# legend-exp/dspeed

Hardware: AMD Instinct MI355X
Metric: waveforms/sec, 4096-sample fp32 trap-energy chain (higher is better)
Workload: dtype f32; 1 GPU; 1000000 x 4096 float32 rows per GPU, fused bl_subtract->pole_zero(tau=1716.28)->trap_filter(625,188)->fixed_time_pickoff('l'); BASELINE configs[1]; rows_per_gpu=1000000, wf_len=4096, device= (gfx950:sramecc+:xnack-), entry=build_processing_chain, kernel=dsp_energy_rr_kernel, lds_bytes_per_wave=19696, waves_per_block=4, blocks=512

## Files before the change

### dspeed_amd/build.py

```python
from __future__ import annotations

import os
import shutil
import subprocess
import sys

HERE = os.path.dirname(os.path.abspath(__file__))
CSRC = os.path.join(HERE, "csrc")
LIB = os.path.join(HERE, "libdspeed_hip.so")
LIB_DIAG = os.path.join(HERE, "libdspeed_hip_diag.so")
SOURCES = ["dsp_vm.hip", "dsp_energy.hip", "dsp_fit.hip", "dsp_rows.hip", "dsp_current.hip", "dsp_scalar.hip", "dsp_reduce.hip", "dsp_pz.hip", "dsp_fir_mfma.hip", "dsp_fir_f16.hip", "dsp_fir_runs.hip", "dsp_plan.cpp", "dsp_host.cpp"]
DEPS = SOURCES + ["dsp_program.h", "dsp_plan.h", "dsp_wave.h", "dsp_reduce_tail.h", os.path.join("..", "..", "include", "dspeed_hip.h")]
FLAGS = ["--offload-arch=gfx950", "-O3", "-std=c++17", "-ffp-contract=off", "-fno-fast-math", "-fPIC", "-shared", "-Wall",
         "-Wno-unused-function"]


NO_SCRATCH = {"dsp_vm.hip": "dsp_vm_kernel"}


def _check_scratch(src: str, remarks: str) -> None:
    frag, name, bad = NO_SCRATCH[src], None, []
    for line in remarks.splitlines():
        if "Function Name:" in line:
            name = line.split("Function Name:")[1].split()[0]
        elif "ScratchSize [bytes/lane]:" in line and name and frag in name:
            n = int(line.split("ScratchSize [bytes/lane]:")[1].split()[0])
            if n:
                bad.append((name, n))
    skip = 0
    for line in remarks.splitlines():
        if "remark:" in line:
            skip = 2
        elif skip and (line.lstrip()[:1].isdigit() or line.lstrip().startswith("|")):
            skip -= 1
        else:
            skip = 0
            sys.stderr.write(line + "\n")
    if bad:
        raise RuntimeError(f"{src}: scratch memory in " + ", ".join(f"{n} ({b} B/lane)" for n, b in bad) +
                           " -- a helper taking Ctx& was outlined, or a local array is indexed at run time (see NO_SCRATCH in build.py)")


def _hipcc() -> str:
    for cand in (os.environ.get("HIPCC"), shutil.which("hipcc"), "/opt/rocm/bin/hipcc"):
        if cand and os.path.exists(cand):
            return cand
    raise RuntimeError("hipcc not found (need ROCm)")


def _stamp(diag: bool) -> str:
    import hashlib

    h = hashlib.sha256(repr((FLAGS, sorted(NO_SCRATCH.items()), diag)).encode())
    for d in DEPS:
        with open(os.path.join(CSRC, d), "rb") as f:
            h.update(d.encode() + b"\0" + f.read())
    return h.hexdigest()


def _stamp_file(lib: str) -> str:
    return lib + ".stamp"


def needs_build(lib: str = LIB) -> bool:
    if not os.path.exists(lib) or not os.path.exists(_stamp_file(lib)):
        return True
    with open(_stamp_file(lib)) as f:
        return f.read().strip() != _stamp(lib == LIB_DIAG)


def build(force: bool = False, verbose: bool = False, diag: bool = False, variant: str | None = None, defines=(), extra_flags=()) -> str:
    lib = LIB_DIAG if diag else LIB
    if variant:
        lib = os.path.join(HERE, f"libdspeed_hip_{variant}.so")
        force = True
    if not force and not needs_build(lib):
        return lib
    objs, procs = [], []
    for src in SOURCES:
        obj = os.path.join(CSRC, "." + src + (f".{variant}.o" if variant else (".diag.o" if diag else ".o")))
        cmd = [_hipcc(), *[f for f in FLAGS if f != "-shared"], *(["-DDSPEED_HIP_DIAG"] if diag else []), *[f"-D{d}" for d in defines], *extra_flags, "-x", "hip", "-c",
               os.path.join(CSRC, src), "-o", obj]
        guard = src in NO_SCRATCH
        if guard:
            cmd.append("-Rpass-analysis=kernel-resource-usage")
        if verbose:
            print(" ".join(cmd))
        procs.append((cmd, subprocess.Popen(cmd, stderr=subprocess.PIPE if guard else None, text=True if guard else None), src))
        objs.append(obj)
    failed = None
    try:
        for cmd, p, src in procs:
            err = p.communicate()[1] if src in NO_SCRATCH else None
            if p.wait() != 0:
                if err:
                    sys.stderr.write(err)
                raise subprocess.CalledProcessError(p.returncode, cmd)
            if err is not None:
                _check_scratch(src, err)
    except BaseException as e:
        failed = e
    if failed is not None:
        for _cmd, p, _src in procs:
            if p.poll() is None:
                p.kill()
            p.wait()
        for obj in objs:
            if os.path.exists(obj):
                os.remove(obj)
        raise failed
    link = [_hipcc(), "--offload-arch=gfx950", "-fPIC", "-shared", *objs, "-o", lib]
    if verbose:
        print(" ".join(link))
    subprocess.check_call(link)
    if variant:
        for obj in objs:
            os.remove(obj)
        return lib
    with open(_stamp_file(lib), "w") as f:
        f.write(_stamp(diag) + "\n")
    return lib


if __name__ == "__main__":
    _variant = sys.argv[sys.argv.index("--variant") + 1] if "--variant" in sys.argv else None
    _defines = [sys.argv[i + 1] for i, a in enumerate(sys.argv[:-1]) if a == "--define"]
    _flags = [sys.argv[i + 1] for i, a in enumerate(sys.argv[:-1]) if a == "--flag"]
    print(build(force="--force" in sys.argv, verbose=True, diag="--diag" in sys.argv, variant=_variant, defines=_defines, extra_flags=_flags))
```

### dspeed_amd/csrc/dsp_energy.hip

```cpp
#include <hip/hip_runtime.h>

#include "dsp_program.h"
#include "dsp_wave.h"

struct EnergyArgs {
    const void* wf;
    int64_t wf_stride;
    int32_t wf_offset;
    int32_t len;
    const float* bl;
    int64_t bl_stride;
    float bl_const;
    int32_t has_bl;
    const float* tp;
    int64_t tp_stride;
    float tp_const;
    int32_t mode;
    float* out;
    int64_t out_stride;
    double c;
    double rr, ll;
    int32_t tau_nan;
    int32_t all_nan;
    int32_t C, pitch;
    float invC;
    int32_t q[3], rho[3];
    int32_t lds_elems_per_wave;
    int32_t slot_off;
    const float* tau;
    int64_t tau_stride;
    int32_t ablate;
};

#ifdef DSPEED_HIP_DIAG
#define ABLATE(A) ((A).ablate)
#else
#define ABLATE(A) 0
#endif

constexpr int rr_prio_after_phase[6] = {1, 2, 3, 3, 3, 0};
#define RR_PRIO_AT(n) __builtin_amdgcn_s_setprio(rr_prio_after_phase[n]);

namespace {

constexpr int G = 8;
constexpr int G3 = 8;

__device__ __forceinline__ unsigned long long stamp() {
    unsigned long long t;
    __builtin_amdgcn_sched_barrier(0);
    asm volatile("s_memtime %0\n\ts_waitcnt lgkmcnt(0)" : "=s"(t)::"memory");
    __builtin_amdgcn_sched_barrier(0);
    return t;
}
#define PHASE(i)                                   \
    if (stamps) {                                  \
        const unsigned long long now_ = stamp();   \
        tsum[i] += now_ - tlast;                   \
        tlast = now_;                              \
    }

template <int N>
__device__ __forceinline__ void load_group(float (&v)[N], const float* p) {
#pragma unroll
    for (int u = 0; u < N; ++u) v[u] = p[u];
}

template <int NPF, int KIND>
__global__ void __launch_bounds__(256, 2) dsp_energy_kernel(EnergyArgs A, int64_t n_wf, int* err) {
    extern __shared__ __attribute__((aligned(16))) unsigned char smem_raw[];
    const int lane = lane_id();
    const double inv_rr = 1.0 / A.rr, inv_ll = 1.0 / A.ll;
    const int wave = __builtin_amdgcn_readfirstlane((int)(threadIdx.x >> 6)), wpb = (int)(blockDim.x >> 6);
    float* lds = reinterpret_cast<float*>(smem_raw) + (size_t)wave * A.lds_elems_per_wave;
    for (int e = lane; e < A.lds_elems_per_wave; e += 64) lds[e] = 0.0f;
    wave_sync();

    constexpr int C = 4 * NPF, pitch = C + 1, len = 256 * NPF;
    float* slot = lds + A.slot_off;
    float* mine = slot + lane * pitch;

    const float* lagp[3];
#pragma unroll
    for (int k = 0; k < 3; ++k) {
        const int jj = lane - A.q[k] - 1;
        lagp[k] = (jj >= -1) ? slot + jj * pitch + (C - A.rho[k]) : slot - 2 * pitch;
    }

    const int64_t stride_rows = (int64_t)gridDim.x * wpb;
    int64_t row = (int64_t)blockIdx.x * wpb + wave;

    typedef float f4 __attribute__((ext_vector_type(4)));
    f4 pf[NPF];
    float pf_bl = 0.0f, pf_tp = 0.0f;
    auto prefetch = [&](int64_t r) {
        const float* g = (const float*)A.wf + r * A.wf_stride + A.wf_offset;
#pragma unroll
        for (int b = 0; b < NPF; ++b) pf[b] = reinterpret_cast<const f4*>(g)[b * 64 + lane];
        pf_bl = A.bl ? A.bl[r * A.bl_stride] : A.bl_const;
        pf_tp = A.tp ? A.tp[r * A.tp_stride] : A.tp_const;
    };
    auto report = [&](int code, int64_t r) {
        if (lane == 0 && atomicCAS(&err[0], 0, code) == 0) {
            err[1] = (int)(r & 0xffffffffll);
            err[2] = (int)(r >> 32);
        }
    };
    if (row < n_wf) prefetch(row);
    const bool stamps = (ABLATE(A) & 8) != 0;
    unsigned long long tsum[6] = {0, 0, 0, 0, 0, 0}, tlast = stamps ? stamp() : 0;

    for (; row < n_wf; row += stride_rows) {
#pragma unroll
        for (int b = 0; b < NPF; ++b) {
            const int e = (b * 64 + lane) * 4;
            float* d = slot + e + e / C;
#pragma unroll
            for (int m = 0; m < 4; ++m) d[m] = pf[b][m];
        }
        const float bl = __int_as_float(__builtin_amdgcn_readfirstlane(__float_as_int(pf_bl)));
        const float t_in = __int_as_float(__builtin_amdgcn_readfirstlane(__float_as_int(pf_tp)));
        const int64_t next = row + stride_rows;
        __builtin_amdgcn_sched_barrier(0);
        if (next < n_wf) prefetch(next);
        __builtin_amdgcn_sched_barrier(0);
        wave_sync();
        PHASE(0)

        float result = quiet_nan<float>();
        double X = 0.0;
        if (!(ABLATE(A) & 1)) {
            float va[G], vb[G];
            load_group(va, mine);
#pragma unroll 1
            for (int t = 0; t < C; t += 2 * G) {
                load_group(vb, mine + t + G);
#pragma unroll
                for (int u = 0; u < G; ++u) X += (double)(va[u] - bl);
                if (t + 2 * G < C) load_group(va, mine + t + 2 * G);
#pragma unroll
                for (int u = 0; u < G; ++u) X += (double)(vb[u] - bl);
            }
        }
// ... 95 lines not shown
                for (int k = 0; k < 4; ++k)
                    if (co[k] >= 0) capmask |= 1u << (co[k] / G3);
                PHASE(3)
                float y = g;
                {
                    float a0[G3], a1[G3], a2[G3], a3[G3], b0[G3], b1[G3], b2[G3], b3[G3];
                    auto fetch = [&](float (&o)[G3], float (&l0)[G3], float (&l1)[G3], float (&l2)[G3], int t) {
                        load_group(o, mine + t);
#pragma unroll
                        for (int k = 0; k < 3; ++k) {
                            float(&dst)[G3] = (k == 0) ? l0 : (k == 1 ? l1 : l2);
                            const int r = A.rho[k];
                            if (t >= r) {
                                load_group(dst, lagp[k] + t + 1);
                            } else if (t + G3 <= r) {
                                load_group(dst, lagp[k] + t);
                            } else {
#pragma unroll
                                for (int u = 0; u < G3; ++u) dst[u] = lagp[k][t + u + ((t + u >= r) ? 1 : 0)];
                            }
                        }
                    };
                    auto body = [&](float (&o)[G3], float (&l0)[G3], float (&l1)[G3], float (&l2)[G3], int t) {
                        float ys[G3];
#pragma unroll
                        for (int u = 0; u < G3; ++u) {
                            y = trap_step_r<float, KIND>(y, o[u], l0[u], l1[u], l2[u], A.rr, A.ll, inv_rr, inv_ll);
                            ys[u] = y;
                        }
                        if ((capmask >> (t / G3)) & 1u) {
#pragma unroll
                            for (int k = 0; k < 4; ++k) {
                                const int d = co[k] - t;
#pragma unroll
                                for (int u = 0; u < G3; ++u)
                                    if (d == u) capv[k] = ys[u];
                            }
                        }
                    };
                    fetch(a0, a1, a2, a3, 0);
#pragma unroll 1
                    for (int t = 0; t < C; t += 2 * G3) {
                        fetch(b0, b1, b2, b3, t + G3);
                        body(a0, a1, a2, a3, t);
                        if (t + 2 * G3 < C) fetch(a0, a1, a2, a3, t + 2 * G3);
                        body(b0, b1, b2, b3, t + G3);
                    }
                }
                PHASE(4)
                const double D = (double)y - (double)g;
                const double delta = wave_exscan_add(D) - (double)g;
                float w4[4];
#pragma unroll
                for (int k = 0; k < 4; ++k) {
                    const float v = (float)((double)capv[k] + delta);
                    w4[k] = cl[k] >= 0 ? readlane(v, cl[k]) : 0.0f;
                }
                int fc = 0;
                result = pickoff_eval(t_in, A.mode, len, w4, fc);
                if (fc) report(fc, row);
            }
        }
        if (lane == 0) A.out[row * A.out_stride] = result;
        wave_sync();
        PHASE(5)
    }
    if (stamps && lane == 0) {
#pragma unroll
        for (int i = 0; i < 6; ++i) atomicAdd(reinterpret_cast<unsigned long long*>(err + 4) + i, tsum[i]);
    }
}

struct EnergyPlan {
    int32_t shift[3][4];
    int32_t cs[3][4];
    int32_t local[3][4];
};

__device__ __attribute__((noinline)) double rr_decay(double tau) { return exp(-1.0 / tau); }

template <int NPF, int KIND, int S, int IN, bool TAU = false>
__global__ void __launch_bounds__(256, NPF >= 32 ? 1 : 2) dsp_energy_rr_kernel(EnergyArgs A, EnergyPlan PL, int64_t n_wf, int* err) {
    extern __shared__ __attribute__((aligned(16))) unsigned char smem_raw[];
    constexpr int C = 4 * NPF + 1, len = 256 * NPF, NG = (C - 1) / 8, CS = (C - 1) / S, NGS = CS / 8;
    constexpr int BS = CS >= 16 ? 16 : CS;
    static_assert((C - 1) % (8 * S) == 0, "sub-chain length must be a whole number of 8-sample groups");
    const int lane = lane_id();
    const double inv_rr = 1.0 / A.rr, inv_ll = 1.0 / A.ll;
    const int wave = __builtin_amdgcn_readfirstlane((int)(threadIdx.x >> 6)), wpb = (int)(blockDim.x >> 6);
    float* lds = reinterpret_cast<float*>(smem_raw) + (size_t)wave * A.lds_elems_per_wave;
    for (int e = lane; e < A.lds_elems_per_wave; e += 64) lds[e] = 0.0f;
    wave_sync();
    float* slot = lds + A.slot_off;
    float* mine = slot + lane * C;
    constexpr int AUXP = NG + 1 <= 9 ? 9 : ((NG + 1) | 1);
    static_assert(NG + 1 <= AUXP && S * NGS + 1 <= AUXP && (AUXP & 1) == 1, "side array too small");
    float* aux = slot + 64 * C + 16 + lane * AUXP;
    const float* lagp[3];
#pragma unroll
    for (int k = 0; k < 3; ++k) {
        const int pos0 = lane * C - A.q[k];
        lagp[k] = (pos0 >= -C) ? slot + pos0 : slot - (2 * C + 8);
    }

    const int64_t stride_rows = (int64_t)gridDim.x * wpb;
    int64_t row = (int64_t)blockIdx.x * wpb + wave;
    typedef float f4 __attribute__((ext_vector_type(4)));
    typedef unsigned int u4 __attribute__((ext_vector_type(4)));
    constexpr int NLD = IN == 0 ? NPF : NPF / 2;
    static_assert(IN == 0 || NPF % 2 == 0, "16-bit rows: an even number of 4-sample groups per lane");
    u4 pf[NLD];
    float pf_bl = 0.0f, pf_tp = 0.0f;
    auto prefetch = [&](int64_t r) {
        const char* g = (const char*)A.wf + (r * A.wf_stride + A.wf_offset) * (IN == 0 ? 4 : 2);
#pragma unroll
        for (int b = 0; b < NLD; ++b) pf[b] = reinterpret_cast<const u4*>(g)[b * 64 + lane];
        typedef const __attribute__((address_space(1))) float* gptr;
        pf_bl = A.bl ? ((gptr)A.bl)[r * A.bl_stride] : A.bl_const;
        pf_tp = A.tp ? ((gptr)A.tp)[r * A.tp_stride] : A.tp_const;
    };
    auto report = [&](int code, int64_t r) {
        if (lane == 0 && atomicCAS(&err[0], 0, code) == 0) {
            err[1] = (int)(r & 0xffffffffll);
            err[2] = (int)(r >> 32);
        }
    };
    if (row < n_wf) prefetch(row);
    const bool stamps = (ABLATE(A) & 8) != 0;
    unsigned long long tsum[6] = {0, 0, 0, 0, 0, 0}, tlast = stamps ? stamp() : 0;
    float pend_result = 0.0f;
    int64_t pend_row = -1;

    for (; row < n_wf; row += stride_rows) {
#pragma unroll
        for (int b = 0; b < NLD; ++b) {
            if (IN == 0) {
                f4 v;
#pragma unroll
                for (int m = 0; m < 4; ++m) v[m] = __uint_as_float(pf[b][m]);
                *reinterpret_cast<f4*>(slot + (b * 64 + lane) * 4) = v - pf_bl;
            } else {
                f4 lo, hi;
#pragma unroll
                for (int m = 0; m < 4; ++m) {
                    const unsigned int wv = pf[b][m];
                    const float s0 = IN == 1 ? (float)(short)(wv & 0xffffu) : (float)(wv & 0xffffu);
                    const float s1 = IN == 1 ? (float)(short)(wv >> 16) : (float)(wv >> 16);
                    if (m < 2) {
                        lo[2 * m] = s0;
                        lo[2 * m + 1] = s1;
                    } else {
                        hi[2 * (m - 2)] = s0;
                        hi[2 * (m - 2) + 1] = s1;
                    }
                }
                *reinterpret_cast<f4*>(slot + (b * 64 + lane) * 8) = lo - pf_bl;
                *reinterpret_cast<f4*>(slot + (b * 64 + lane) * 8 + 4) = hi - pf_bl;
            }
        }
        slot[len + lane] = 0.0f;
        const float t_in = __int_as_float(__builtin_amdgcn_readfirstlane(__float_as_int(pf_tp)));
        const int64_t next = row + stride_rows;
        __builtin_amdgcn_sched_barrier(0);
        if (next < n_wf) prefetch(next);
        if (pend_row >= 0 && lane == 0) A.out[pend_row * A.out_stride] = pend_result;
        __builtin_amdgcn_sched_barrier(0);
        wave_sync();
        PHASE(0)
        RR_PRIO_AT(0)

        float result = quiet_nan<float>();
        float xr[C];
#pragma unroll
        for (int t = 0; t < C; ++t) xr[t] = mine[t];
        const float xprev = (lane > 0) ? mine[-1] : 0.0f;
        double Xp[4] = {0.0, 0.0, 0.0, 0.0};
#pragma unroll
        for (int t = 0; t < C; ++t) {
            if ((t & 7) == 0) __builtin_amdgcn_sched_barrier(0);
            Xp[t & 3] += (double)xr[t];
        }
        const double X = (Xp[0] + Xp[1]) + (Xp[2] + Xp[3]);
        double c_row = A.c;
        bool in_nan = A.tau_nan != 0;
        if constexpr (TAU) {
            const float tau = A.tau[row * A.tau_stride];
            in_nan = tau != tau;
            c_row = rr_decay((double)tau);
        }
        if (wave_any(!(fabs(X) <= 1.7976931348623157e308))) {
            bool n = false;
#pragma unroll
            for (int t = 0; t < C; ++t) n |= (xr[t] != xr[t]);
            in_nan |= wave_any(n);
        }
        PHASE(1)
        RR_PRIO_AT(1)
#pragma unroll
        for (int t = 0; t < C; ++t) asm volatile("" : "+v"(xr[t]));
        if (!in_nan) {
            const double E = wave_exscan_add(X);
            const double c = c_row;
            double xp = (double)xprev, acc = E - c * (E - xp);
            float run = 0.0f;
#pragma unroll
            for (int t = 0; t < C; ++t) {
                if ((t & 7) == 0) __builtin_amdgcn_sched_barrier(0);
                const double x = (double)xr[t];
                acc += __builtin_fma(-c, xp, x);
                const float y = (float)acc;
                xr[t] = y;
                mine[t] = y;
                xp = x;
                run += y;
                if ((t & 7) == 7) aux[t >> 3] = run;
            }
            wave_sync();
            PHASE(2)
        RR_PRIO_AT(2)
            bool pz_nan = false;
            if (wave_any(!(fabsf(run) <= 3.4028234663852886e38f))) {
                bool n = false;
#pragma unroll
                for (int t = 0; t < C; ++t) n |= (xr[t] != xr[t]);
                pz_nan = wave_any(n);
            }
            if (pz_nan) {
                report(DSP_E_PZ_NAN, row);
            } else if (!A.all_nan && !(ABLATE(A) & 4) && pickoff_in_range(t_in, len)) {
                const double Ep = wave_exscan_add((double)run);
                float g[S], y[S];
#pragma unroll
                for (int s = 0; s < S; ++s) {
                    double Ak[3];
                    float pbase[3], pv[3][8];
                    int pn[3];
#pragma unroll
                    for (int k = 0; k < 3; ++k) {
                        int r = PL.cs[k][s] * CS + PL.local[k][s];
                        asm volatile("" : "+s"(r));
                        const int gi = (r > 0 ? r - 1 : 0) >> 3;
                        pn[k] = r - 8 * gi;
                        const float b = aux[gi > 0 ? gi - 1 : 0];
                        pbase[k] = gi > 0 ? b : 0.0f;
                        const float* p = mine + 8 * gi;
#pragma unroll
                        for (int u = 0; u < 8; ++u) pv[k][u] = p[u];
                    }
#pragma unroll
                    for (int k = 0; k < 3; ++k) {
                        float part = 0.0f;
#pragma unroll
                        for (int u = 0; u < 8; ++u) part += (u < pn[k]) ? pv[k][u] : 0.0f;
                        Ak[k] = wave_shift_up(Ep + (double)(pbase[k] + part), PL.shift[k][s]);
                    }
                    const double own = Ep + (s ? (double)aux[s * NGS - 1] : 0.0);
                    double Gd;
                    if (KIND == TRAP_FILTER)
                        Gd = ((own - Ak[0]) - Ak[1]) + Ak[2];
                    else if (KIND == TRAP_NORM)
                        Gd = (((own - Ak[0]) - Ak[1]) + Ak[2]) / A.rr;
                    else
                        Gd = (own - Ak[0]) / A.rr - (Ak[1] - Ak[2]) / A.ll;
                    g[s] = (lane == 0 && s == 0) ? -0.0f : (float)Gd;
                    y[s] = g[s];
                }
                PHASE(3)
        RR_PRIO_AT(3)
                wave_sync();
                const int i0 = (int)t_in;
                int capst[2], capoff[2], caplane[2];
#pragma unroll
                for (int k = 0; k < 2; ++k) {
                    const int e = i0 + k;
                    const bool ok = e >= 0 && e < len;
                    caplane[k] = ok ? e / C : 0;
                    capoff[k] = ok ? e - caplane[k] * C : 0;
                    capst[k] = ok ? capoff[k] / BS : -1;
                }
                int capmask = (capst[0] >= 0 ? 1 << capst[0] : 0) | (capst[1] >= 0 ? 1 << capst[1] : 0);
                asm volatile("" : "+s"(capmask));
                float* capbuf = slot + 64 * C + 16 + 64 * AUXP;
                float ysb[S][BS];
                constexpr int GL = 4, NL = CS / GL;
                constexpr int PD = S == 1 ? 2 : 1;
                float lb[PD + 1][S][GL][3], lodd[3] = {0.0f, 0.0f, 0.0f};
#pragma unroll
                for (int p = 0; p < PD; ++p)
#pragma unroll
                    for (int s = 0; s < S; ++s)
#pragma unroll
                        for (int u = 0; u < GL; ++u)
#pragma unroll
                            for (int k = 0; k < 3; ++k) lb[p][s][u][k] = lagp[k][s * CS + p * GL + u];
#pragma unroll
                for (int gl = 0; gl < NL; ++gl) {
                    __builtin_amdgcn_sched_barrier(0);
                    if (gl + PD < NL) {
#pragma unroll
                        for (int s = 0; s < S; ++s)
#pragma unroll
                            for (int u = 0; u < GL; ++u)
#pragma unroll
                                for (int k = 0; k < 3; ++k) lb[(gl + PD) % (PD + 1)][s][u][k] = lagp[k][s * CS + (gl + PD) * GL + u];
                    } else if (gl + PD == NL) {
#pragma unroll
                        for (int k = 0; k < 3; ++k) lodd[k] = lagp[k][C - 1];
                    }
                    if ((gl * GL) % 8 == 0) {
#pragma unroll
                        for (int s = 0; s < S; ++s) aux[s * NGS + (gl * GL) / 8] = y[s];
                    }
                    __builtin_amdgcn_sched_barrier(0);
#pragma unroll
                    for (int u = 0; u < GL; ++u)
#pragma unroll
                        for (int s = 0; s < S; ++s) {
                            y[s] = trap_step_r<float, KIND>(y[s], xr[s * CS + gl * GL + u], lb[gl % (PD + 1)][s][u][0], lb[gl % (PD + 1)][s][u][1],
                                                          lb[gl % (PD + 1)][s][u][2], A.rr, A.ll, inv_rr, inv_ll);
                            ysb[s][(gl * GL + u) % BS] = y[s];
                        }
                    if (((gl + 1) * GL) % BS == 0) {
#pragma unroll
                        for (int s = 0; s < S; ++s) {
                            const int q = s * (CS / BS) + (gl * GL) / BS;
                            if (capmask & (1 << q)) {
#pragma unroll
                                for (int k = 0; k < 2; ++k)
                                    if (capst[k] == q && lane == caplane[k]) {
#pragma unroll
                                        for (int u = 0; u < BS; ++u) capbuf[k * 16 + u] = ysb[s][u];
                                    }
                            }
                        }
                    }
                }
                aux[S * NGS] = y[S - 1];
                y[S - 1] = trap_step_r<float, KIND>(y[S - 1], xr[C - 1], lodd[0], lodd[1], lodd[2], A.rr, A.ll, inv_rr, inv_ll);
                PHASE(4)
        RR_PRIO_AT(4)
                double D[S], Dbefore[S], Dtot = 0.0;
#pragma unroll
                for (int s = 0; s < S; ++s) {
                    D[s] = (double)y[s] - (double)g[s];
                    Dbefore[s] = Dtot;
                    Dtot += D[s];
                }
                const double T0 = wave_exscan_add(Dtot);
                const bool wide = (A.mode == 'h');
                float w4[4];
#pragma unroll
                for (int k = 0; k < 2; ++k) {
                    float v = capbuf[k * 16 + (capoff[k] % BS)];
                    v = capoff[k] == C - 1 ? y[S - 1] : v;
                    double delta = T0 - (double)g[0];
#pragma unroll
                    for (int s = 1; s < S; ++s)
                        if (capoff[k] >= s * CS) delta = (T0 + Dbefore[s]) - (double)g[s];
                    w4[1 + k] = capst[k] >= 0 ? readlane((float)((double)v + delta), caplane[k]) : 0.0f;
                }
#pragma unroll
                for (int k = 0; k < 4; k += 3) {
                    const int e = i0 - 1 + k;
                    const bool need = wide && e >= 0 && e < len;
                    w4[k] = 0.0f;
                    __builtin_amdgcn_sched_barrier(0);
                    if (need) {
                        const int l = e / C, off = e - l * C;
                        int ch = off / CS;
                        if (ch > S - 1) ch = S - 1;
                        const int loc = off - ch * CS;
                        const int gi = loc >> 3, u0 = loc & 7;
                        float ys = aux[ch * NGS + gi], gsel = 0.0f;
                        double dsel = 0.0;
#pragma unroll
                        for (int s = 0; s < S; ++s)
                            if (ch == s) {
                                gsel = g[s];
                                dsel = Dbefore[s];
                            }
                        const int base = ch * CS + gi * 8;
                        float yk = ys;
#pragma unroll
                        for (int u = 0; u < 8; ++u) {
                            const int tt = base + u;
                            ys = trap_step_r<float, KIND>(ys, mine[tt], lagp[0][tt], lagp[1][tt], lagp[2][tt], A.rr, A.ll, inv_rr, inv_ll);
                            if (u == u0) yk = ys;
                        }
                        const double delta = (T0 + dsel) - (double)gsel;
                        w4[k] = readlane((float)((double)yk + delta), l);
                    }
                }
                int fc = 0;
                result = pickoff_eval(t_in, A.mode, len, w4, fc);
                if (fc) report(fc, row);
            }
        }
        pend_result = result;
        pend_row = row;
        wave_sync();
        PHASE(5)
        RR_PRIO_AT(5)
    }
    if (pend_row >= 0 && lane == 0) A.out[pend_row * A.out_stride] = pend_result;
    if (stamps && lane == 0) {
#pragma unroll
        for (int i = 0; i < 6; ++i) atomicAdd(reinterpret_cast<unsigned long long*>(err + 4) + i, tsum[i]);
    }
}

template <int KIND, int S, int IN, bool TAU = false>
int launch_rr_kind(const EnergyArgs& A, const EnergyPlan& PL, int npf, int64_t n_wf, int* err, int blocks, int threads, int lds_bytes,
                   hipStream_t st) {
    switch (npf) {
        case 4: hipLaunchKernelGGL((dsp_energy_rr_kernel<4, KIND, S, IN, TAU>), dim3(blocks), dim3(threads), lds_bytes, st, A, PL, n_wf, err); break;
        case 8: hipLaunchKernelGGL((dsp_energy_rr_kernel<8, KIND, S, IN, TAU>), dim3(blocks), dim3(threads), lds_bytes, st, A, PL, n_wf, err); break;
        case 16: hipLaunchKernelGGL((dsp_energy_rr_kernel<16, KIND, S, IN, TAU>), dim3(blocks), dim3(threads), lds_bytes, st, A, PL, n_wf, err); break;
        case 32:
            if (S != 1) return (int)hipErrorInvalidValue;
            hipLaunchKernelGGL((dsp_energy_rr_kernel<32, KIND, 1, IN, TAU>), dim3(blocks), dim3(threads), lds_bytes, st, A, PL, n_wf, err);
            break;
        default: return (int)hipErrorInvalidValue;
    }
    return (int)hipGetLastError();
}

template <int KIND>
int launch_kind(const EnergyArgs& A, int npf, int64_t n_wf, int* err, int blocks, int threads, int lds_bytes, hipStream_t s) {
    switch (npf) {
        case 4: hipLaunchKernelGGL((dsp_energy_kernel<4, KIND>), dim3(blocks), dim3(threads), lds_bytes, s, A, n_wf, err); break;
        case 8: hipLaunchKernelGGL((dsp_energy_kernel<8, KIND>), dim3(blocks), dim3(threads), lds_bytes, s, A, n_wf, err); break;
        case 16: hipLaunchKernelGGL((dsp_energy_kernel<16, KIND>), dim3(blocks), dim3(threads), lds_bytes, s, A, n_wf, err); break;
        case 32: hipLaunchKernelGGL((dsp_energy_kernel<32, KIND>), dim3(blocks), dim3(threads), lds_bytes, s, A, n_wf, err); break;
        default: return (int)hipErrorInvalidValue;
    }
    return (int)hipGetLastError();
}

}

extern "C" int dsp_internal_launch_energy(const EnergyArgs* A, int trap_opcode, int npf, int64_t n_wf, int* err, int blocks,
                                          int threads, int lds_bytes, hipStream_t stream) {
    if (trap_opcode == DSP_OP_TRAP_FILTER) return launch_kind<TRAP_FILTER>(*A, npf, n_wf, err, blocks, threads, lds_bytes, stream);
    if (trap_opcode == DSP_OP_TRAP_NORM) return launch_kind<TRAP_NORM>(*A, npf, n_wf, err, blocks, threads, lds_bytes, stream);
    return launch_kind<TRAP_ASYM>(*A, npf, n_wf, err, blocks, threads, lds_bytes, stream);
}

extern "C" int dsp_internal_set_energy_lds(int trap_opcode, int npf, int lds_bytes) {
#define SET_(NPF, KIND)                                                                                                   \
    if (npf == NPF && kind == KIND)                                                                                        \
        return (int)hipFuncSetAttribute(reinterpret_cast<const void*>(&dsp_energy_kernel<NPF, KIND>),                      \
                                        hipFuncAttributeMaxDynamicSharedMemorySize, lds_bytes);
    const int kind = trap_opcode == DSP_OP_TRAP_FILTER ? TRAP_FILTER : (trap_opcode == DSP_OP_TRAP_NORM ? TRAP_NORM : TRAP_ASYM);
    SET_(4, TRAP_FILTER) SET_(8, TRAP_FILTER) SET_(16, TRAP_FILTER) SET_(32, TRAP_FILTER)
    SET_(4, TRAP_NORM) SET_(8, TRAP_NORM) SET_(16, TRAP_NORM) SET_(32, TRAP_NORM)
    SET_(4, TRAP_ASYM) SET_(8, TRAP_ASYM) SET_(16, TRAP_ASYM) SET_(32, TRAP_ASYM)
#undef SET_
    return (int)hipErrorInvalidValue;
}

extern "C" int dsp_internal_launch_energy_rr(const EnergyArgs* A, const EnergyPlan* PL, int trap_opcode, int npf, int S, int wf_dtype,
                                             int64_t n_wf, int* err, int blocks, int threads, int lds_bytes, hipStream_t stream) {
#define GO_(KIND)                                                                                                          \
    if (A->tau && wf_dtype == DSP_I16) return launch_rr_kind<KIND, 1, 1, true>(*A, *PL, npf, n_wf, err, blocks, threads, lds_bytes, stream); \
    if (A->tau && wf_dtype == DSP_U16) return launch_rr_kind<KIND, 1, 2, true>(*A, *PL, npf, n_wf, err, blocks, threads, lds_bytes, stream); \
    if (A->tau) return launch_rr_kind<KIND, 1, 0, true>(*A, *PL, npf, n_wf, err, blocks, threads, lds_bytes, stream);       \
    if (wf_dtype == DSP_I16) return launch_rr_kind<KIND, 1, 1>(*A, *PL, npf, n_wf, err, blocks, threads, lds_bytes, stream); \
    if (wf_dtype == DSP_U16) return launch_rr_kind<KIND, 1, 2>(*A, *PL, npf, n_wf, err, blocks, threads, lds_bytes, stream); \
    return S == 2 ? launch_rr_kind<KIND, 2, 0>(*A, *PL, npf, n_wf, err, blocks, threads, lds_bytes, stream)                \
// ... 10 lines not shown
```

### dspeed_amd/csrc/dsp_plan.cpp

```cpp
#include "dsp_plan.h"

#include <algorithm>
#include <cmath>
#include <cstdarg>
#include <cstdio>
#include <cstdlib>
#include <cstring>
#include <memory>
#include <vector>

namespace {
thread_local std::string g_last_error;
}

int dsp_fail(int code, const char* fmt, ...) {
    char buf[512];
    va_list ap;
    va_start(ap, fmt);
    vsnprintf(buf, sizeof buf, fmt, ap);
    va_end(ap);
    g_last_error = buf;
    return code;
}
void dsp_set_last_error(const char* text) { g_last_error = text ? text : ""; }
// ... 1257 lines not shown
        }
    }
    P.n_ops = n_dev_ops;

    {
        int i = 0;
        const dsp_op* ld = (n_ops > i && ops[i].opcode == DSP_OP_LOAD) ? &ops[i++] : nullptr;
        const dsp_op* bs = (ld && n_ops > i && ops[i].opcode == DSP_OP_BL_SUBTRACT) ? &ops[i++] : nullptr;
        const dsp_op* pz = (ld && n_ops > i && ops[i].opcode == DSP_OP_POLE_ZERO) ? &ops[i++] : nullptr;
        const dsp_op* tp = (pz && n_ops > i && ops[i].opcode == DSP_OP_TRAP_PICKOFF) ? &ops[i++] : nullptr;
        const dsp_op* st = (tp && n_ops > i && ops[i].opcode == DSP_OP_STORE_SCALAR) ? &ops[i++] : nullptr;
        const int wdt = ld ? io[ld->io].dtype : -1;
        const bool tau_col = pz && pz->sp[0].kind == DSP_ARG_INPUT && io[pz->sp[0].index].dtype == DSP_F32;
        const bool shape = !f64 && st && i == n_ops && n_slots == 1 && ld->ip[0] == 0 && ld->ip[1] == 0 && (wdt == DSP_F32 || wdt == DSP_I16 || wdt == DSP_U16) && P.io[ld->io].vec_ok &&
                           (!bs || (bs->dst == 0 && bs->src == 0 && bs->sp[0].kind != DSP_ARG_REG)) && pz->dst == 0 && pz->src == 0 &&
                           (pz->sp[0].kind == DSP_ARG_CONST || tau_col) &&
                           tp->src == 0 && tp->sp[0].kind != DSP_ARG_REG && st->ip[0] == tp->dst &&
                           (slot_len[0] == 1024 || slot_len[0] == 2048 || slot_len[0] == 4096 || slot_len[0] == 8192);
        if (!shape && st && i == n_ops && n_slots == 1) {
            if (f64) note(ch, "the energy chain in a float64 loop: the fused energy kernels are float32");
            else if (pz->sp[0].kind != DSP_ARG_CONST && !tau_col)
                note(ch, "a pole-zero time constant per event that is not a float32 column: the fused energy kernels take a constant or such a column");
            else if (!(slot_len[0] == 1024 || slot_len[0] == 2048 || slot_len[0] == 4096 || slot_len[0] == 8192))
                note(ch, "waveforms of %d samples: the fused energy kernels take 1024, 2048, 4096 or 8192", slot_len[0]);
            else if (!P.io[ld->io].vec_ok) note(ch, "rows that do not start on 16-byte boundaries: the fused energy kernels read 16 bytes per lane");
        }
        auto f32_col = [&](const dsp_scalar_arg& a) { return a.kind != DSP_ARG_INPUT || io[a.index].dtype == DSP_F32; };
        if (shape && (!bs || f32_col(bs->sp[0])) && f32_col(tp->sp[0]) && io[st->io].dtype == DSP_F32) {
            EnergyArgs& F = ch->fused;
            const DevOp& dpz = P.ops[dev_index[pz - ops]];
            const DevOp& dtp = P.ops[dev_index[tp - ops]];
            F.wf_stride = io[ld->io].row_stride;
            F.wf_offset = io[ld->io].offset;
            F.len = slot_len[0];
            F.has_bl = bs ? 1 : 0;
            if (bs) {
                if (bs->sp[0].kind == DSP_ARG_INPUT) {
                    ch->io_bl = bs->sp[0].index;
                    F.bl_stride = io[ch->io_bl].row_stride;
                } else {
                    F.bl_const = (float)bs->sp[0].value;
                }
            }
            if (tp->sp[0].kind == DSP_ARG_INPUT) {
                ch->io_tp = tp->sp[0].index;
                F.tp_stride = io[ch->io_tp].row_stride;
            } else {
                F.tp_const = (float)tp->sp[0].value;
            }
            F.mode = tp->io;
            F.out_stride = io[st->io].row_stride;
            F.c = dpz.fc[0];
            F.tau_nan = dpz.ic[0];
            F.rr = dtp.fc[0];
            F.ll = dtp.fc[1];
            F.all_nan = dtp.ic[9];
            F.C = P.slots[0].C;
            F.pitch = P.slots[0].pitch;
            F.invC = P.slots[0].invC;
            for (int k = 0; k < 3; ++k) {
                F.q[k] = dtp.ic[3 + k];
                F.rho[k] = dtp.ic[6 + k];
            }
            F.lds_elems_per_wave = P.lds_elems_per_wave;
            F.slot_off = P.slots[0].off;
#ifdef DSPEED_HIP_DIAG
            if (const char* ab = getenv("DSPEED_HIP_ABLATE")) F.ablate = atoi(ab);
#endif
            ch->io_wf = ld->io;
            ch->io_out = st->io;
            ch->fused_trap = tp->ip[3];
            ch->fused_npf = slot_len[0] / 256;
            ch->fused_ok = slot_len[0] <= 4096 && wdt == DSP_F32 && !tau_col;
            if (tau_col) {
                ch->io_tau = pz->sp[0].index;
                F.tau_stride = io[ch->io_tau].row_stride;
            }
            ch->wf_dtype = wdt;
            const char* env = getenv("DSPEED_HIP_NO_FUSED");
            ch->fused_on = !(env && env[0] == '1');
            {
                EnergyArgs& I = ch->rr;
                I = F;
                const int Ci = slot_len[0] / 64 + 1;
                I.C = Ci;
                I.pitch = Ci;
                I.invC = 1.0f / (float)Ci;
                int guard = 2 * Ci + 8;
                guard = ((guard + 3) / 4) * 4;
                I.slot_off = guard;
                const int ng1 = (Ci - 1) / 8 + 1, auxp = ng1 <= 9 ? 9 : (ng1 | 1);
                int elems = guard + 64 * Ci + 16 + 64 * auxp + 32;
                elems = ((elems + 3) / 4) * 4;
                I.lds_elems_per_wave = elems;
                ch->rr_lds_bytes = elems * 4;
                for (int k = 0; k < 3; ++k) {
                    I.q[k] = dtp.ic[k];
                    I.rho[k] = 0;
                }
                for (int S = 1; S <= 2; ++S) {
                    const int CS = (Ci - 1) / S;
                    for (int k = 0; k < 3; ++k)
                        for (int sidx = 0; sidx < S; ++sidx) {
                            const int pos = sidx * CS - dtp.ic[k];
                            const int r = ((pos % Ci) + Ci) % Ci;
                            const int shift = (r - pos) / Ci;
                            int cs = r / CS;
                            if (cs > S - 1) cs = S - 1;
                            ch->plan[S - 1].shift[k][sidx] = shift;
                            ch->plan[S - 1].cs[k][sidx] = cs;
                            ch->plan[S - 1].local[k][sidx] = r - cs * CS;
                        }
                }
                ch->rr_ok = true;
                ch->variant = 6;
                if (const char* venv = getenv("DSPEED_HIP_VARIANT")) ch->variant = atoi(venv);
                if (ch->variant != 1 && ch->variant != 8) ch->variant = 6;
            }
        }
    }

    ch->fir_ok = match_fir_shape(ch, ops, n_ops, io, slot_len, n_slots, f64);
    if (!ch->fir_ok) {
        for (int k = 0; k < DSP_FIR_MAXK; ++k) ch->fio_taps[k] = ch->fio_out[k] = -1;
        ch->fir_ok = match_fir_store_shape(ch, ops, n_ops, io, slot_len, n_slots, f64);
    }
    if (ch->fir_ok) {
        const char* env = getenv("DSPEED_HIP_NO_FUSED");
        ch->fused_on = !(env && env[0] == '1');
        const char* f32 = getenv("DSPEED_HIP_FIR_F32");
        const dsp_io_desc& w = io[ch->fio_wf];
        const int es = w.dtype == DSP_F32 ? 4 : 2;
        const int n_slice = ch->fir.n;
        if (!(f32 && f32[0] == '1') && (w.row_stride * es) % 16 == 0 && (w.offset * es) % 16 == 0 &&
            ((n_slice & 7) == 0 || w.offset + ((n_slice + 7) & ~7) <= w.row_stride)) {
            ch->fir_f16 = true;
            ch->f16.tz = dsp_internal_fir_f16_tz(ch->fir.kend);
        }
    }
    ch->rows_ok = match_rows_shape(ch, ops, n_ops, io, n_io, slot_len, n_slots, dev_index, f64);
    if (!ch->rows_ok) {
        ch->rio_wf = ch->rio_bl = ch->rio_thr = ch->rio_ts = ch->rio_tpt = ch->rio_dwt = -1;
        for (int k = 0; k < 4; ++k) ch->rio_mm[k] = -1;
    } else {
        const char* env = getenv("DSPEED_HIP_NO_FUSED");
        ch->fused_on = !(env && env[0] == '1');
    }

    {
        bool only_scalar = true;
        for (int i = 0; i < n_ops; ++i) {
            const int oc = ops[i].opcode;
            only_scalar &= oc == DSP_OP_SCALAR_AFFINE || oc == DSP_OP_SCALAR_DIV || oc == DSP_OP_SCALAR_CONVERT || oc == DSP_OP_SCALAR_FUNC ||
                           oc == DSP_OP_STORE_SCALAR;
        }
        ch->scalar_ok = only_scalar && n_dev_ops == n_ops;
        if (ch->scalar_ok) {
            const char* env = getenv("DSPEED_HIP_NO_FUSED");
            ch->fused_on = !(env && env[0] == '1');
        }
    }
    ch->pz_ok = match_pz_rows_shape(ch, ops, n_ops, io, slot_len, n_slots, dev_index, f64);
    if (ch->pz_ok) {
        const char* env = getenv("DSPEED_HIP_NO_FUSED");
        ch->fused_on = !(env && env[0] == '1');
    }
    ch->red_ok = match_reduce_shape(ch, ops, n_ops, io, slot_len, f64);
    if (ch->red_ok) {
        const char* env = getenv("DSPEED_HIP_NO_FUSED");
        ch->fused_on = !(env && env[0] == '1');
    }
    {
        const char* off = getenv("DSPEED_HIP_NO_FIR_RUNS");
        if (!ch->red_ok && !(off && off[0] == '1')) ch->runs_ok = match_fir_runs_shape(ch, ops, n_ops, io, slot_len, n_slots, f64);
        if (ch->runs_ok) {
            const char* env = getenv("DSPEED_HIP_NO_FUSED");
            ch->fused_on = !(env && env[0] == '1');
            ch->fir_ok = ch->fir_f16 = false;
        }
    }
    ch->cur_ok = match_current_shape(ch, ops, n_ops, io, slot_len, f64);
    if (!ch->cur_ok) {
        ch->cio_wf = ch->cio_t0 = -1;
        for (int k = 0; k < 4; ++k) ch->cio_out[k] = -1;
// ... 240 lines not shown
```

Before: 340.3 million waveforms/s.

## Pad per-lane LDS pitch to even and use 8-byte LDS accesses in rr kernel

Changes the per-lane chunk pitch in LDS from 4*NPF+1 to 4*NPF+2 so each lane's samples are 8-byte aligned, then reads and writes samples as float2 pairs instead of single floats. Lagged trapezoid-filter reads are re-based to even addresses, and the replay loop is specialised at compile time for each combination of lag parities. A compiler barrier keeps adjacent pairs from being merged into ds_read2/ds_write2, and a build-time disassembly check enforces that. The aim is to halve LDS instruction count in the recursive filter phases, at the cost of one extra virtual sample per lane, slightly more LDS, more template instantiations, and a possible change in bank-conflict behaviour with the even pitch.

```diff
diff --git a/dspeed_amd/build.py b/dspeed_amd/build.py
--- a/dspeed_amd/build.py
+++ b/dspeed_amd/build.py
@@ -41,6 +41,53 @@
                            " -- a helper taking Ctx& was outlined, or a local array is indexed at run time (see NO_SCRATCH in build.py)")
 
 
+RR_NO_FUSED_LDS = {"dsp_energy.hip": ("dsp_energy_rr_kernel", ("ds_read2_b64", "ds_write2_b64"),
+                                      "RR_NO_MERGE no longer keeps neighbouring 8-byte LDS accesses apart (see dsp_energy.hip)")}
+
+
+def _llvm_tool(name: str) -> str | None:
+    roots = [os.path.join(os.path.dirname(os.path.dirname(os.path.realpath(_hipcc()))), "llvm", "bin"),
+             os.path.join(os.path.dirname(os.path.realpath(_hipcc())), "..", "lib", "llvm", "bin"), "/opt/rocm/llvm/bin"]
+    for r in roots:
+        if os.path.exists(os.path.join(r, name)):
+            return os.path.join(r, name)
+    return shutil.which(name)
+
+
+def _check_instructions(src: str, obj: str) -> None:
+    import re
+    import tempfile
+
+    frag, barred, why = RR_NO_FUSED_LDS[src]
+    tools = [_llvm_tool(t) for t in ("llvm-objcopy", "clang-offload-bundler", "llvm-objdump")]
+    if os.environ.get("DSPEED_HIP_NO_ISA_CHECK") == "1":
+        sys.stderr.write(f"{src}: instruction check skipped (DSPEED_HIP_NO_ISA_CHECK=1)\n")
+        return
+    if None in tools:
+        raise RuntimeError(f"{src}: cannot check the kernels' instructions: llvm-objcopy / clang-offload-bundler / llvm-objdump not found beside "
+                           "hipcc's clang or on PATH (they ship with ROCm's LLVM; DSPEED_HIP_NO_ISA_CHECK=1 builds without the check)")
+    objcopy, bundler, objdump = tools
+    with tempfile.TemporaryDirectory() as tmp:
+        fat, co = os.path.join(tmp, "fatbin"), os.path.join(tmp, "gfx950.co")
+        subprocess.check_call([objcopy, f"--dump-section=.hip_fatbin={fat}", obj, os.path.join(tmp, "copy.o")])
+        subprocess.check_call([bundler, "--unbundle", "--type=o", "--targets=hipv4-amdgcn-amd-amdhsa--gfx950", f"--input={fat}", f"--output={co}"])
+        asm = subprocess.run([objdump, "-d", co], check=True, stdout=subprocess.PIPE, text=True).stdout
+    name, seen, bad = None, 0, {}
+    for line in asm.splitlines():
+        m = re.match(r"^[0-9a-f]+ <(\S+)>:", line)
+        if m:
+            name = m.group(1) if frag in m.group(1) else None
+            seen += name is not None
+        elif name:
+            for op in barred:
+                if re.search(rf"\b{op}\b", line):
+                    bad[name] = bad.get(name, 0) + 1
+    if not seen:
+        raise RuntimeError(f"{src}: no {frag} in the disassembly -- the instruction check looks at nothing (RR_NO_FUSED_LDS in build.py)")
+    if bad:
+        raise RuntimeError(f"{src}: {' / '.join(barred)} in " + ", ".join(f"{n} ({c})" for n, c in sorted(bad.items())) + f" -- {why}")
+
+
 def _hipcc() -> str:
     for cand in (os.environ.get("HIPCC"), shutil.which("hipcc"), "/opt/rocm/bin/hipcc"):
         if cand and os.path.exists(cand):
@@ -51,7 +98,7 @@
 def _stamp(diag: bool) -> str:
     import hashlib
 
-    h = hashlib.sha256(repr((FLAGS, sorted(NO_SCRATCH.items()), diag)).encode())
+    h = hashlib.sha256(repr((FLAGS, sorted(NO_SCRATCH.items()), sorted(RR_NO_FUSED_LDS.items()), diag)).encode())
     for d in DEPS:
         with open(os.path.join(CSRC, d), "rb") as f:
             h.update(d.encode() + b"\0" + f.read())
@@ -98,6 +145,8 @@
                 raise subprocess.CalledProcessError(p.returncode, cmd)
             if err is not None:
                 _check_scratch(src, err)
+            if src in RR_NO_FUSED_LDS:
+                _check_instructions(src, objs[SOURCES.index(src)])
     except BaseException as e:
         failed = e
     if failed is not None:
diff --git a/dspeed_amd/csrc/dsp_energy.hip b/dspeed_amd/csrc/dsp_energy.hip
--- a/dspeed_amd/csrc/dsp_energy.hip
+++ b/dspeed_amd/csrc/dsp_energy.hip
@@ -1,4 +1,6 @@
 #include <hip/hip_runtime.h>
+
+#include <type_traits>
 
 #include "dsp_program.h"
 #include "dsp_wave.h"
@@ -41,6 +43,8 @@
 constexpr int rr_prio_after_phase[6] = {1, 2, 3, 3, 3, 0};
 #define RR_PRIO_AT(n) __builtin_amdgcn_s_setprio(rr_prio_after_phase[n]);
 
+#define RR_NO_MERGE() asm volatile("" ::: "memory")
+
 namespace {
 
 constexpr int G = 8;
@@ -59,6 +63,8 @@
         tsum[i] += now_ - tlast;                   \
         tlast = now_;                              \
     }
+
+constexpr int rr_pair_lo(int st, int par, int np) { return st == 0 ? 0 : (2 * st + par < np ? 2 * st + par : np); }
 
 template <int N>
 __device__ __forceinline__ void load_group(float (&v)[N], const float* p) {
@@ -320,9 +326,11 @@
 template <int NPF, int KIND, int S, int IN, bool TAU = false>
 __global__ void __launch_bounds__(256, NPF >= 32 ? 1 : 2) dsp_energy_rr_kernel(EnergyArgs A, EnergyPlan PL, int64_t n_wf, int* err) {
     extern __shared__ __attribute__((aligned(16))) unsigned char smem_raw[];
-    constexpr int C = 4 * NPF + 1, len = 256 * NPF, NG = (C - 1) / 8, CS = (C - 1) / S, NGS = CS / 8;
+    constexpr int C = 4 * NPF + 2, len = 256 * NPF, NG = (C - 2) / 8, CS = (C - 2) / S, NGS = CS / 8;
     constexpr int BS = CS >= 16 ? 16 : CS;
-    static_assert((C - 1) % (8 * S) == 0, "sub-chain length must be a whole number of 8-sample groups");
+    static_assert((C - 2) % (8 * S) == 0, "sub-chain length must be a whole number of 8-sample groups");
+    static_assert(C % 2 == 0 && 64 * C - len == 128, "even pitch: 8-byte aligned lane chunks, two rows of virtual samples above len");
+    typedef float f2 __attribute__((ext_vector_type(2)));
     const int lane = lane_id();
     const double inv_rr = 1.0 / A.rr, inv_ll = 1.0 / A.ll;
     const int wave = __builtin_amdgcn_readfirstlane((int)(threadIdx.x >> 6)), wpb = (int)(blockDim.x >> 6);
@@ -331,14 +339,17 @@
     wave_sync();
     float* slot = lds + A.slot_off;
     float* mine = slot + lane * C;
+    f2* mine2 = reinterpret_cast<f2*>(mine);
     constexpr int AUXP = NG + 1 <= 9 ? 9 : ((NG + 1) | 1);
     static_assert(NG + 1 <= AUXP && S * NGS + 1 <= AUXP && (AUXP & 1) == 1, "side array too small");
     float* aux = slot + 64 * C + 16 + lane * AUXP;
-    const float* lagp[3];
+    const float* lagb[3];
+    int lagpar[3];
 #pragma unroll
     for (int k = 0; k < 3; ++k) {
-        const int pos0 = lane * C - A.q[k];
-        lagp[k] = (pos0 >= -C) ? slot + pos0 : slot - (2 * C + 8);
+        lagpar[k] = A.q[k] & 1;
+        const int pos0 = lane * C - A.q[k] - lagpar[k];
+        lagb[k] = (pos0 + lagpar[k] >= -C) ? slot + pos0 : slot - (2 * C + 8);
     }
 
     const int64_t stride_rows = (int64_t)gridDim.x * wpb;
@@ -396,7 +407,7 @@
                 *reinterpret_cast<f4*>(slot + (b * 64 + lane) * 8 + 4) = hi - pf_bl;
             }
         }
-        slot[len + lane] = 0.0f;
+        reinterpret_cast<f2*>(slot + len)[lane] = f2{0.0f, 0.0f};
         const float t_in = __int_as_float(__builtin_amdgcn_readfirstlane(__float_as_int(pf_tp)));
         const int64_t next = row + stride_rows;
         __builtin_amdgcn_sched_barrier(0);
@@ -410,7 +421,12 @@
         float result = quiet_nan<float>();
         float xr[C];
 #pragma unroll
-        for (int t = 0; t < C; ++t) xr[t] = mine[t];
+        for (int j = 0; j < C / 2; ++j) {
+            const f2 v = mine2[j];
+            RR_NO_MERGE();
+            xr[2 * j] = v.x;
+            xr[2 * j + 1] = v.y;
+        }
         const float xprev = (lane > 0) ? mine[-1] : 0.0f;
         double Xp[4] = {0.0, 0.0, 0.0, 0.0};
 #pragma unroll
@@ -448,7 +464,10 @@
                 acc += __builtin_fma(-c, xp, x);
                 const float y = (float)acc;
                 xr[t] = y;
-                mine[t] = y;
+                if (t & 1) {
+                    mine2[t >> 1] = f2{xr[t - 1], y};
+                    RR_NO_MERGE();
+                }
                 xp = x;
                 run += y;
                 if ((t & 7) == 7) aux[t >> 3] = run;
@@ -481,9 +500,14 @@
                         pn[k] = r - 8 * gi;
                         const float b = aux[gi > 0 ? gi - 1 : 0];
                         pbase[k] = gi > 0 ? b : 0.0f;
-                        const float* p = mine + 8 * gi;
-#pragma unroll
-                        for (int u = 0; u < 8; ++u) pv[k][u] = p[u];
+                        const f2* p = mine2 + 4 * gi;
+#pragma unroll
+                        for (int u = 0; u < 4; ++u) {
+                            const f2 v = p[u];
+                            RR_NO_MERGE();
+                            pv[k][2 * u] = v.x;
+                            pv[k][2 * u + 1] = v.y;
+                        }
                     }
 #pragma unroll
                     for (int k = 0; k < 3; ++k) {
@@ -519,62 +543,96 @@
                 int capmask = (capst[0] >= 0 ? 1 << capst[0] : 0) | (capst[1] >= 0 ? 1 << capst[1] : 0);
                 asm volatile("" : "+s"(capmask));
                 float* capbuf = slot + 64 * C + 16 + 64 * AUXP;
-                float ysb[S][BS];
-                constexpr int GL = 4, NL = CS / GL;
-                constexpr int PD = S == 1 ? 2 : 1;
-                float lb[PD + 1][S][GL][3], lodd[3] = {0.0f, 0.0f, 0.0f};
-#pragma unroll
-                for (int p = 0; p < PD; ++p)
-#pragma unroll
-                    for (int s = 0; s < S; ++s)
+                float ytail[2];
+                auto replay = [&](auto p0, auto p1, auto p2) __attribute__((always_inline)) {
+                    constexpr int par[3] = {decltype(p0)::value, decltype(p1)::value, decltype(p2)::value};
+                    constexpr int GL = 4, NL = CS / GL;
+                    constexpr int PD = S == 1 && NPF < 32 ? 2 : 1;
+                    constexpr int NPS = CS / 2 + 2;
+                    f2 lp[3][S][NPS];
+                    const f2* lagb2[3] = {reinterpret_cast<const f2*>(lagb[0]), reinterpret_cast<const f2*>(lagb[1]), reinterpret_cast<const f2*>(lagb[2])};
+                    float ysb[S][BS];
+                    auto load_stage = [&](int st) __attribute__((always_inline)) {
+#pragma unroll
+                        for (int s = 0; s < S; ++s)
+#pragma unroll
+                            for (int jj = 0; jj < 3; ++jj)
+#pragma unroll
+                                for (int k = 0; k < 3; ++k) {
+                                    const int np = (CS + (s == S - 1 ? 2 : 0) + par[k] + 1) / 2;
+                                    const int j = rr_pair_lo(st, par[k], np) + jj;
+                                    if (j < rr_pair_lo(st + 1, par[k], np)) {
+                                        lp[k][s][j] = lagb2[k][s * (CS / 2) + j];
+                                        RR_NO_MERGE();
+                                    }
+                                }
+                    };
+                    auto lagged = [&](int k, int s, int t) __attribute__((always_inline)) { return lp[k][s][(t + par[k]) >> 1][(t + par[k]) & 1]; };
+#pragma unroll
+                    for (int st = 0; st < PD; ++st) load_stage(st);
+#pragma unroll
+                    for (int gl = 0; gl < NL; ++gl) {
+                        __builtin_amdgcn_sched_barrier(0);
+                        load_stage(gl + PD);
+                        if ((gl * GL) % 8 == 0) {
+#pragma unroll
+                            for (int s = 0; s < S; ++s) aux[s * NGS + (gl * GL) / 8] = y[s];
+                        }
+                        __builtin_amdgcn_sched_barrier(0);
 #pragma unroll
                         for (int u = 0; u < GL; ++u)
 #pragma unroll
-                            for (int k = 0; k < 3; ++k) lb[p][s][u][k] = lagp[k][s * CS + p * GL + u];
-#pragma unroll
-                for (int gl = 0; gl < NL; ++gl) {
-                    __builtin_amdgcn_sched_barrier(0);
-                    if (gl + PD < NL) {
-#pragma unroll
-                        for (int s = 0; s < S; ++s)
-#pragma unroll
-                            for (int u = 0; u < GL; ++u)
-#pragma unroll
-                                for (int k = 0; k < 3; ++k) lb[(gl + PD) % (PD + 1)][s][u][k] = lagp[k][s * CS + (gl + PD) * GL + u];
-                    } else if (gl + PD == NL) {
-#pragma unroll
-                        for (int k = 0; k < 3; ++k) lodd[k] = lagp[k][C - 1];
-                    }
-                    if ((gl * GL) % 8 == 0) {
-#pragma unroll
-                        for (int s = 0; s < S; ++s) aux[s * NGS + (gl * GL) / 8] = y[s];
-                    }
-                    __builtin_amdgcn_sched_barrier(0);
-#pragma unroll
-                    for (int u = 0; u < GL; ++u)
-#pragma unroll
-                        for (int s = 0; s < S; ++s) {
-                            y[s] = trap_step_r<float, KIND>(y[s], xr[s * CS + gl * GL + u], lb[gl % (PD + 1)][s][u][0], lb[gl % (PD + 1)][s][u][1],
-                                                          lb[gl % (PD + 1)][s][u][2], A.rr, A.ll, inv_rr, inv_ll);
-                            ysb[s][(gl * GL + u) % BS] = y[s];
-                        }
-                    if (((gl + 1) * GL) % BS == 0) {
-#pragma unroll
-                        for (int s = 0; s < S; ++s) {
-                            const int q = s * (CS / BS) + (gl * GL) / BS;
-                            if (capmask & (1 << q)) {
-#pragma unroll
-                                for (int k = 0; k < 2; ++k)
-                                    if (capst[k] == q && lane == caplane[k]) {
-#pragma unroll
-                                        for (int u = 0; u < BS; ++u) capbuf[k * 16 + u] = ysb[s][u];
-                                    }
+                            for (int s = 0; s < S; ++s) {
+                                const int t = gl * GL + u;
+                                y[s] = trap_step_r<float, KIND>(y[s], xr[s * CS + t], lagged(0, s, t), lagged(1, s, t), lagged(2, s, t), A.rr, A.ll, inv_rr, inv_ll);
+                                ysb[s][t % BS] = y[s];
                             }
-                        }
-                    }
-                }
-                aux[S * NGS] = y[S - 1];
-                y[S - 1] = trap_step_r<float, KIND>(y[S - 1], xr[C - 1], lodd[0], lodd[1], lodd[2], A.rr, A.ll, inv_rr, inv_ll);
+                        if (((gl + 1) * GL) % BS == 0) {
+#pragma unroll
+                            for (int s = 0; s < S; ++s) {
+                                const int q = s * (CS / BS) + (gl * GL) / BS;
+                                if (capmask & (1 << q)) {
+#pragma unroll
+                                    for (int k = 0; k < 2; ++k)
+                                        if (capst[k] == q && lane == caplane[k]) {
+#pragma unroll
+                                            for (int u = 0; u < BS; ++u) capbuf[k * 16 + u] = ysb[s][u];
+                                        }
+                                }
+                            }
+                        }
+                    }
+                    aux[S * NGS] = y[S - 1];
+#pragma unroll
+                    for (int u = 0; u < 2; ++u) {
+                        y[S - 1] = trap_step_r<float, KIND>(y[S - 1], xr[C - 2 + u], lagged(0, S - 1, CS + u), lagged(1, S - 1, CS + u), lagged(2, S - 1, CS + u),
+                                                          A.rr, A.ll, inv_rr, inv_ll);
+                        ytail[u] = y[S - 1];
+                    }
+                };
+                {
+                    typedef std::integral_constant<int, 0> E;
+                    typedef std::integral_constant<int, 1> O;
+                    if constexpr (KIND == TRAP_ASYM) {
+                        switch (lagpar[0] | (lagpar[1] << 1) | (lagpar[2] << 2)) {
+                            case 0: replay(E{}, E{}, E{}); break;
+                            case 1: replay(O{}, E{}, E{}); break;
+                            case 2: replay(E{}, O{}, E{}); break;
+                            case 3: replay(O{}, O{}, E{}); break;
+                            case 4: replay(E{}, E{}, O{}); break;
+                            case 5: replay(O{}, E{}, O{}); break;
+                            case 6: replay(E{}, O{}, O{}); break;
+                            default: replay(O{}, O{}, O{}); break;
+                        }
+                    } else {
+                        switch (lagpar[0] | (lagpar[1] << 1)) {
+                            case 0: replay(E{}, E{}, E{}); break;
+                            case 1: replay(O{}, E{}, O{}); break;
+                            case 2: replay(E{}, O{}, O{}); break;
+                            default: replay(O{}, O{}, E{}); break;
+                        }
+                    }
+                }
                 PHASE(4)
         RR_PRIO_AT(4)
                 double D[S], Dbefore[S], Dtot = 0.0;
@@ -590,7 +648,7 @@
 #pragma unroll
                 for (int k = 0; k < 2; ++k) {
                     float v = capbuf[k * 16 + (capoff[k] % BS)];
-                    v = capoff[k] == C - 1 ? y[S - 1] : v;
+                    v = capoff[k] >= C - 2 ? (capoff[k] == C - 2 ? ytail[0] : ytail[1]) : v;
                     double delta = T0 - (double)g[0];
 #pragma unroll
                     for (int s = 1; s < S; ++s)
@@ -622,7 +680,8 @@
 #pragma unroll
                         for (int u = 0; u < 8; ++u) {
                             const int tt = base + u;
-                            ys = trap_step_r<float, KIND>(ys, mine[tt], lagp[0][tt], lagp[1][tt], lagp[2][tt], A.rr, A.ll, inv_rr, inv_ll);
+                            ys = trap_step_r<float, KIND>(ys, mine[tt], lagb[0][tt + lagpar[0]], lagb[1][tt + lagpar[1]], lagb[2][tt + lagpar[2]], A.rr, A.ll,
+                                                          inv_rr, inv_ll);
                             if (u == u0) yk = ys;
                         }
                         const double delta = (T0 + dsel) - (double)gsel;
diff --git a/dspeed_amd/csrc/dsp_plan.cpp b/dspeed_amd/csrc/dsp_plan.cpp
--- a/dspeed_amd/csrc/dsp_plan.cpp
+++ b/dspeed_amd/csrc/dsp_plan.cpp
@@ -1363,14 +1363,14 @@
             {
                 EnergyArgs& I = ch->rr;
                 I = F;
-                const int Ci = slot_len[0] / 64 + 1;
+                const int Ci = slot_len[0] / 64 + 2;
                 I.C = Ci;
                 I.pitch = Ci;
                 I.invC = 1.0f / (float)Ci;
                 int guard = 2 * Ci + 8;
                 guard = ((guard + 3) / 4) * 4;
                 I.slot_off = guard;
-                const int ng1 = (Ci - 1) / 8 + 1, auxp = ng1 <= 9 ? 9 : (ng1 | 1);
+                const int ng1 = (Ci - 2) / 8 + 1, auxp = ng1 <= 9 ? 9 : (ng1 | 1);
                 int elems = guard + 64 * Ci + 16 + 64 * auxp + 32;
                 elems = ((elems + 3) / 4) * 4;
                 I.lds_elems_per_wave = elems;
@@ -1380,7 +1380,7 @@
                     I.rho[k] = 0;
                 }
                 for (int S = 1; S <= 2; ++S) {
-                    const int CS = (Ci - 1) / S;
+                    const int CS = (Ci - 2) / S;
                     for (int k = 0; k < 3; ++k)
                         for (int sidx = 0; sidx < S; ++sidx) {
                             const int pos = sidx * CS - dtp.ic[k];
```

Measured after the change: 347.3 million waveforms/s (median of 6 runs). 2.1% higher.
